# dojo-sim/Dojo.jl

Hardware: NVIDIA H100
Metric: env-steps/sec (forward step!) (higher is better)
Workload: dtype f64

## Files before the change

dojo.jl_b200/csrc/dojo_b200.cu:

```cuda
#include <cuda_runtime.h>

#include <algorithm>
#include <climits>
#include <cstdio>
#include <cstdlib>
#include <cstring>
#include <string>
#include <vector>

#include "../../include/dojo_b200.h"
#include "dojo_step_kernel.cuh"
#include "dojo_kin.cuh"
#include "dojo_kinjac.cuh"
#include "dojo_envs.cuh"
#include "dojo_storage.cuh"

using namespace dj;

extern "C" __attribute__((visibility("hidden"))) const void* dojo_cm_step_kernel(int grad);
static const void* step_kernel_fn(bool any_contact, bool grad, bool plan_smem, bool small = false) {
  if (any_contact) return dojo_cm_step_kernel(grad ? 1 : 0);
  if (plan_smem && !getenv("DOJO_B200_GENERIC_PLAN")) {
    if (!grad && small) return (const void*)dojo_step_kernel<false, true, false, true>;
    return grad ? (const void*)dojo_step_kernel<true, true> : (const void*)dojo_step_kernel<false, true>;
// ... 447 lines not shown
            gfold.push_back(joints[j].gv_off);
          }
        const BodyDev& B = bodies[b];
        const JointDev& J = joints[pj[b]];
        {
          HStep h; std::memset(&h, 0, sizeof(h));
          ElimStep& s = h.s;
          s.d_off = B.D_off; s.n = 6; s.vec_off = B.sol_off; s.r_off = B.r_off; s.nnb = 0;
          s.fold_off = (int)ilist.size(); s.fold_cnt = (int)fold.size();
          for (int f : fold) ilist.push_back(f);
          s.gfold_off = (int)ilist.size();
          for (int f : gfold) ilist.push_back(f);
          int ij = -1, ip = -1;
          if (joint_nq(J) > 0) {
            ij = s.nnb++;
            s.nb[ij].n = joint_nq(J); s.nb[ij].vec_off = J.sol_off; s.nb[ij].r_off = J.r_off; s.nb[ij].gv_off = -1; s.nb[ij].fwd_abs = -1; s.nb[ij].L_off = J.Uc_off; s.nb[ij].U_off = J.Lc_off; s.nb[ij].U_k = 6; s.nb[ij].U_row = 0;
            s.nb[ij].ld = joint_nq(J); s.nb[ij].row0 = 0;
          }
          int r0 = 0;
          if (J.parent >= 0 && J.BBpc_off >= 0) {
            ip = s.nnb++;
            const BodyDev& Pb = bodies[J.parent];
            r0 = (J.flags & JF_FULL) ? 0 : 3;
            s.nb[ip].n = 6 - r0; s.nb[ip].vec_off = Pb.sol_off + r0; s.nb[ip].r_off = Pb.r_off + r0; s.nb[ip].gv_off = J.gv_off; s.nb[ip].fwd_abs = J.S_off + 36 + r0;
            s.nb[ip].L_off = J.BBpc_off; s.nb[ip].U_off = J.BBcp_off; s.nb[ip].U_k = 6 - r0; s.nb[ip].U_row = r0;
            s.nb[ip].ld = 6; s.nb[ip].row0 = r0;
          }
          if (ij >= 0) s.tgt[ij][ij] = J.D_off;
          if (ip >= 0) s.tgt[ip][ip] = J.S_off + 7 * r0;
          if (ij >= 0 && ip >= 0) { s.tgt[ij][ip] = J.Up_off + r0; s.tgt[ip][ij] = J.Lp_off + r0 * joint_nq(J); }
          h.height = hb; h.group = -1; h.cost = 4.0 + joint_nq(J) * 0.3;
          hs.push_back(h);
        }
        int hj = hb;
        if (joint_nq(J) > 0) {
          HStep h; std::memset(&h, 0, sizeof(h));
          ElimStep& s = h.s;
          s.d_off = J.D_off; s.n = joint_nq(J); s.vec_off = J.sol_off; s.r_off = J.r_off; s.nnb = 0;
          if (J.parent >= 0) {
            const BodyDev& Pb = bodies[J.parent];
            s.nnb = 1;
            s.nb[0].n = 6; s.nb[0].vec_off = Pb.sol_off; s.nb[0].r_off = Pb.r_off; s.nb[0].gv_off = J.gv_off; s.nb[0].fwd_abs = J.S_off + 36; s.nb[0].L_off = J.Lp_off; s.nb[0].U_off = J.Up_off; s.nb[0].U_k = joint_nq(J); s.nb[0].U_row = 0;
            s.nb[0].ld = 6; s.nb[0].row0 = 0;
            s.tgt[0][0] = J.S_off;
          }
          hj = hb + 1;
          h.height = hj; h.group = -1; h.cost = 2.0 + joint_nq(J) * 0.4;
          hs.push_back(h);
        }
        return hj;
      }
    } rec{joints, bodies, contacts, parent_joint, done, hs, ilist, Ne, Ni};
    for (int j = 0; j < Ne; ++j) if (joints[j].parent < 0 && !done[joints[j].child]) rec.visit(joints[j].child);
    for (int b = 0; b < Nb; ++b) if (!done[b]) { delete h; return fail("mechanism is not a tree rooted at the origin"); }
  }
  int nphase = 0;
  for (auto& x : hs) nphase = std::max(nphase, x.height + 1);
  std::vector<ElimStep> steps;
  std::vector<int> sched((size_t)nphase * nw * 2, 0);
  for (int ph = 0; ph < nphase; ++ph) {
    std::vector<std::vector<int>> per_warp(nw);
    std::vector<double> load(nw, 0.0);
    std::vector<int> group_warp(Nb, -1);
    for (int i = 0; i < (int)hs.size(); ++i) {
      if (hs[i].height != ph) continue;
      int w;
      if (hs[i].group >= 0 && group_warp[hs[i].group] >= 0) w = group_warp[hs[i].group];
      else {
        w = 0;
        for (int k = 1; k < nw; ++k) if (load[k] < load[w]) w = k;
        if (hs[i].group >= 0) group_warp[hs[i].group] = w;
      }
      per_warp[w].push_back(i);
      load[w] += hs[i].cost;
    }
    for (int w = 0; w < nw; ++w) {
      sched[2 * (ph * nw + w)] = (int)steps.size();
      sched[2 * (ph * nw + w) + 1] = (int)per_warp[w].size();
      for (int i : per_warp[w]) steps.push_back(hs[i].s);
    }
  }
  P.nphase = nphase;
  h->nsteps = (int)steps.size();

  cudaDeviceProp prop;
  if (cudaGetDeviceProperties(&prop, device) != cudaSuccess) { delete h; g_create_error = "cudaGetDeviceProperties failed"; return DOJO_ECUDA; }
  h->sm_count = prop.multiProcessorCount;
  if (h->arena_bytes > (size_t)prop.sharedMemPerBlockOptin) {
    delete h;
    g_create_error = "dojo_create: mechanism does not fit the per-environment shared-memory arena";
    return DOJO_ENOMEM;
  }
  auto upload = [&](const void* src, size_t bytes, void** dst) -> bool {
    if (bytes == 0) { *dst = nullptr; return true; }
    if (cudaMalloc(dst, bytes) != cudaSuccess) return false;
    return cudaMemcpy(*dst, src, bytes, cudaMemcpyHostToDevice) == cudaSuccess;
  };
  std::vector<char> blob;
  {
    const void* src[8] = {bodies.data(), joints.data(), contacts.data(), steps.data(), sched.data(), ilist.data(), roles.data(), ucol.data()};
    const size_t len[8] = {sizeof(BodyDev) * Nb, sizeof(JointDev) * Ne, sizeof(ContactDev) * Ni, sizeof(ElimStep) * steps.size(), sizeof(int) * sched.size(),
                           sizeof(int) * ilist.size(), sizeof(WarpRole) * roles.size(), sizeof(int) * ucol.size()};
    const int order[8] = {3, 4, 5, 6, 7, 0, 2, 1};
    for (int q = 0; q < 8; ++q) {
      const int k = order[q];
      h->blob_off[k] = (int)blob.size();
      blob.insert(blob.end(), (const char*)src[k], (const char*)src[k] + len[k]);
      blob.resize((blob.size() + 15) & ~size_t(15), 0);
      h->blob_end[k] = (int)blob.size();
    }
    h->blob_bytes = (int)blob.size();
  }
  bool ok = upload(blob.data(), blob.size(), (void**)&h->d_blob);
  {
    std::vector<int> order;
    std::vector<char> placed(Nb, 0), used(Ne, 0);
    for (bool progress = true; progress && (int)order.size() < Ne;) {
      progress = false;
      for (int j = 0; j < Ne; ++j)
        if (!used[j] && (joints[j].parent < 0 || placed[joints[j].parent])) { order.push_back(j); used[j] = 1; placed[joints[j].child] = 1; progress = true; }
    }
    ok = ok && (int)order.size() == Ne && upload(order.data(), sizeof(int) * Ne, (void**)&h->d_kin_order);
  }
  ok = ok && cudaMalloc((void**)&h->d_counter, sizeof(int)) == cudaSuccess;
  ok = ok && cudaMalloc((void**)&h->d_order, sizeof(int) * max_batch) == cudaSuccess && cudaMalloc((void**)&h->d_prev_iters, sizeof(int32_t) * max_batch) == cudaSuccess &&
       cudaMemset(h->d_prev_iters, 0, sizeof(int32_t) * max_batch) == cudaSuccess;
  if (const char* e = getenv("DOJO_B200_LPT")) { h->lpt = atoi(e) != 0; h->lpt_mode = atoi(e); }
  ok = ok && cudaMalloc((void**)&h->d_key, sizeof(int32_t) * max_batch) == cudaSuccess;
  ok = ok && cudaMalloc((void**)&h->d_prof, (32 + 2 * (size_t)max_batch) * sizeof(unsigned long long)) == cudaSuccess && cudaMemset(h->d_prof, 0, 32 * sizeof(unsigned long long)) == cudaSuccess &&
       cudaMemset(h->d_prof + 31, 0xff, sizeof(unsigned long long)) == cudaSuccess;
  ok = ok && cudaStreamCreateWithFlags(&h->stream, cudaStreamNonBlocking) == cudaSuccess;
  ok = ok && cudaEventCreateWithFlags(&h->ev_last, cudaEventDisableTiming) == cudaSuccess;
  auto pick_slots = [&](size_t bytes) {
    int g = (int)std::min<size_t>((size_t)prop.sharedMemPerBlockOptin / bytes, (size_t)(256 / (32 * nw)));
    g = std::max(1, std::min(g, 8));
    if (const char* e = getenv("DOJO_B200_SLOTS")) { int v = atoi(e); if (v >= 1 && v <= g) g = v; }
    return g;
  };
  h->slots = pick_slots(h->arena_bytes);
  const bool smem_plan = !getenv("DOJO_B200_GLOBAL_PLAN");
  auto plan_prefix = [&](int n, size_t bytes, int* off, int* pbytes, int* mask) {
    *off = -1; *pbytes = 0; *mask = 0;
    if (!smem_plan) return;
    const size_t room = (size_t)prop.sharedMemPerBlockOptin - 1024 - n * bytes;
    for (int k = 0; k < 8; ++k)
      if ((size_t)h->blob_end[k] <= room) { *mask |= 1 << k; *pbytes = std::max(*pbytes, h->blob_end[k]); }
    for (int k = 0; k < 8; ++k)
      if (((*mask >> k) & 1) && h->blob_end[k] > *pbytes) *mask &= ~(1 << k);
    if (*mask) *off = (int)(n * bytes / sizeof(double));
  };
  plan_prefix(h->slots, h->arena_bytes, &h->plan_smem_off, &h->plan_smem_bytes, &h->plan_smem_mask);
  h->smem_fwd = h->slots * h->arena_bytes + h->plan_smem_bytes;
  h->small_step = small_step_ok(h, h->plan_smem_mask);
  h->k_fwd = step_kernel_fn(h->any_contact, false, h->plan_smem_mask == 0xff, h->small_step);
  h->k_grad = step_kernel_fn(h->any_contact, true, false);
  ok = ok && max_shared_memory(h->k_fwd, device) == cudaSuccess;
  const bool grad_fits = h->grad_bytes <= (size_t)prop.sharedMemPerBlockOptin;
  if (grad_fits) {
    h->slots_grad = pick_slots(h->grad_bytes);
    plan_prefix(h->slots_grad, h->grad_bytes, &h->plan_smem_off_grad, &h->plan_smem_bytes_grad, &h->plan_smem_mask_grad);
    h->smem_grad = h->slots_grad * h->grad_bytes + h->plan_smem_bytes_grad;
    h->k_grad = step_kernel_fn(h->any_contact, true, h->plan_smem_mask_grad == 0xff);
    ok = ok && max_shared_memory(h->k_grad, device) == cudaSuccess;
  } else h->grad_bytes = 0;
  if (!ok) { g_create_error = std::string("dojo_create: device allocation failed: ") + cudaGetErrorString(cudaGetLastError()); dojo_destroy(h); return DOJO_ECUDA; }
  P.bodies = (const BodyDev*)(h->d_blob + h->blob_off[0]); P.joints = (const JointDev*)(h->d_blob + h->blob_off[1]);
  P.contacts = (const ContactDev*)(h->d_blob + h->blob_off[2]); P.steps = (const ElimStep*)(h->d_blob + h->blob_off[3]);
  P.sched = (const int*)(h->d_blob + h->blob_off[4]); P.ilist = (const int*)(h->d_blob + h->blob_off[5]);
  P.roles = (const WarpRole*)(h->d_blob + h->blob_off[6]); P.ucol = (const int*)(h->d_blob + h->blob_off[7]);
  int occ = 1;
  cudaOccupancyMaxActiveBlocksPerMultiprocessor(&occ, h->k_fwd, 32 * h->nw * h->slots, h->smem_fwd);
  h->envs_per_sm = std::max(1, occ);
  if (h->grad_bytes) { occ = 1; cudaOccupancyMaxActiveBlocksPerMultiprocessor(&occ, h->k_grad, 32 * h->nw * h->slots_grad, h->smem_grad); h->envs_per_sm_grad = std::max(1, occ); }
  *out = h;
  return DOJO_OK;
}

extern "C" int dojo_destroy(DojoHandle* h) {
  if (!h) return DOJO_OK;
  cudaSetDevice(h->device);
  cudaFree(h->d_key); cudaFree(h->d_order); cudaFree(h->d_prev_iters); cudaFree(h->d_prof); cudaFree(h->d_blob); cudaFree(h->d_counter); cudaFree(h->d_kin_order); cudaFree(h->d_kjws); cudaFree(h->d_kjout); cudaFree(h->d_recZ[0]); cudaFree(h->d_recZ[1]); cudaFree(h->d_recS); cudaFree(h->d_recD); cudaFree(h->d_recAny); cudaFree(h->d_envTheta); cudaFree(h->d_envNorm); cudaFree(h->d_envS); cudaFree(h->d_envSn); cudaFree(h->d_envA); cudaFree(h->d_envR); cudaFree(h->d_envS0); cudaFree(h->d_envDone); cudaFree(h->d_X); cudaFree(h->d_Xn); cudaFree(h->d_gsol); cudaFree(h->d_gstatus); cudaFree(h->d_done); cudaFree(h->d_trace);
  for (int k = 0; k < 2; ++k) { cudaFree(h->d_Fz[k]); cudaFree(h->d_Fu[k]); if (h->ev_kernel[k]) cudaEventDestroy(h->ev_kernel[k]); if (h->ev_copy[k]) cudaEventDestroy(h->ev_copy[k]); }
  if (h->copy_stream) cudaStreamDestroy(h->copy_stream);
  cudaFree(h->d_Z); cudaFree(h->d_U); cudaFree(h->d_F); cudaFree(h->d_Zn); cudaFree(h->d_sol); cudaFree(h->d_status); cudaFree(h->d_iters);
  if (h->p_in) cudaFreeHost(h->p_in);
  if (h->p_out) cudaFreeHost(h->p_out);
// ... 1245 lines not shown
```

dojo.jl_b200/csrc/dojo_kernels.cuh:

```cuda
#pragma once
#include "dojo_linalg.cuh"
#include "dojo_plan.h"

namespace dj {

#ifdef DJ_ANY_CONTACT
#define DJ_SLOT_OFF(raw) ((raw) & 0x3fffffff)
#define DJ_SLOT_FULL(raw) (((raw) >> 30) & 1)
#else
#define DJ_SLOT_OFF(raw) (raw)
#endif
#ifdef DJ_ANY_CONTACT
DJ_DEV int contact_type(const ContactDev& cd) { return cd.tn & 0xff; }
DJ_DEV int contact_nh(const ContactDev& cd) { return cd.tn >> 8; }
#endif

DJ_DEV V3 ld3(const double* p) { return V3{p[0], p[1], p[2]}; }
DJ_DEV void st3(double* p, V3 v) { p[0] = v.x; p[1] = v.y; p[2] = v.z; }
DJ_DEV void add3(double* p, V3 v) { p[0] += v.x; p[1] += v.y; p[2] += v.z; }
DJ_DEV M33 ldm33(const double* p) {
  M33 r;
#pragma unroll
  for (int i = 0; i < 3; ++i)
#pragma unroll
    for (int j = 0; j < 3; ++j) r.m[i][j] = p[3 * i + j];
  return r;
}
DJ_DEV void stm33(double* p, const M33& a) {
#pragma unroll
  for (int i = 0; i < 3; ++i)
#pragma unroll
    for (int j = 0; j < 3; ++j) p[3 * i + j] = a.m[i][j];
}
DJ_DEV Quat ldq(const double* p) { return Quat{p[0], p[1], p[2], p[3]}; }

struct Ctx {
  double* A;
  const Plan* P;
  const BodyDev* bodies;
  const JointDev* joints;
  const ContactDev* contacts;
  const ElimStep* steps;
  const int* sched;
  const int* ilist;
  const WarpRole* roles;
  const int* ucol;
  int tid, nthreads, warp, lane;
  int sd;
  int bar;
  double mu;
  int slot, nslots, slot_stride;
  double* arena0;
  int* s_int;
  double* s_dbl;
  int apar, assist;
#ifdef DJ_PROFILE
  long long t_eval_jac, t_eval_ls, t_fact, t_solve, t_misc, t_align, t_cone, t_center, t_rolewait, t_last;
  long long f_fold, f_inv, f_rm, f_schur, f_bar, f_last;
#endif
};
#ifdef DJ_PROFILE
#define DJ_TICK(c, field) { long long _t = clock64(); (c).field += _t - (c).t_last; (c).t_last = _t; }
#define DJ_FTICK(c, field) { long long _t = clock64(); (c).field += _t - (c).f_last; (c).f_last = _t; }
#else
#define DJ_TICK(c, field) {}
#define DJ_FTICK(c, field) {}
#endif

#ifdef DJ_HOSTEMU
DJ_DEV void slot_sync(const Ctx& c) { hostemu_bar_sync(c.bar, c.nthreads); }
#else
DJ_DEV void slot_sync(const Ctx& c) { asm volatile("bar.sync %0, %1;" ::"r"(c.bar), "r"(c.nthreads) : "memory"); }
#endif

constexpr int kMaxAssistTrials = 16;
struct AlignInfo { int n_live, owner; };
#ifdef DJ_HOSTEMU
DJ_DEV void cta_barrier() { __syncthreads(); }
#else
__device__ __noinline__ void cta_barrier() { __syncthreads(); }
#endif
DJ_DEV AlignInfo cta_align(Ctx& c, bool live) {
  int* fl = c.s_int + 8 + 8 * c.apar;
  c.apar ^= 1;
  if (c.tid == 0) fl[c.slot] = live ? 1 : 0;
  cta_barrier();
  AlignInfo r;
  r.n_live = 0; r.owner = -1;
  for (int q = 0; q < c.nslots; ++q)
    if (fl[q]) { r.n_live++; r.owner = q; }
  return r;
}
DJ_DEV void assist_release(Ctx& c) {
  if (!c.assist) return;
  if (c.tid == 0) c.s_int[24] = 0;
  cta_barrier();
  c.assist = 0;
}

template <bool SMALL>
DJ_DEV int slot_warps(const Ctx& c) { return SMALL ? 2 : c.P->nw; }

template <bool SMALL = false>
DJ_DEV void block_nanmax2(const Ctx& c, double& a, double& b) {
  double* red = c.A + c.P->red_off;
  a = warp_nanmax(a);
  b = warp_nanmax(b);
  if (slot_warps<SMALL>(c) == 1) return;
  if (c.lane == 0) { red[2 * c.warp] = a; red[2 * c.warp + 1] = b; }
  slot_sync(c);
  a = red[0]; b = red[1];
  for (int w = 1; w < slot_warps<SMALL>(c); ++w) { a = nanmax(a, red[2 * w]); b = nanmax(b, red[2 * w + 1]); }
  slot_sync(c);
}
template <bool SMALL = false>
DJ_DEV double block_min(const Ctx& c, double a) {
  double* red = c.A + c.P->red_off;
  a = warp_min(a);
  if (slot_warps<SMALL>(c) == 1) return a;
  if (c.lane == 0) red[c.warp] = a;
  slot_sync(c);
  a = red[0];
  for (int w = 1; w < slot_warps<SMALL>(c); ++w) a = fmin(a, red[w]);
  slot_sync(c);
  return a;
}
template <bool SMALL = false>
DJ_DEV void block_sum3(const Ctx& c, double& a, double& b, double& d) {
  double* red = c.A + c.P->red_off;
  a = warp_sum(a); b = warp_sum(b); d = warp_sum(d);
  if (slot_warps<SMALL>(c) == 1) return;
  if (c.lane == 0) { red[3 * c.warp] = a; red[3 * c.warp + 1] = b; red[3 * c.warp + 2] = d; }
  slot_sync(c);
  a = red[0]; b = red[1]; d = red[2];
  for (int w = 1; w < slot_warps<SMALL>(c); ++w) { a += red[3 * w]; b += red[3 * w + 1]; d += red[3 * w + 2]; }
  slot_sync(c);
}

DJ_DEV int role_item(const WarpRole& r, int p, int lane) { return lane < r.count[p] ? r.first[p] + lane : -1; }

struct Kin {
// ... 941 lines not shown
      const double* s = A + DJ_SLOT_OFF(c.ilist[bd.g_off + g]);
      add3(rb, ld3(s));
      add3(rb + 3, ld3(s + 3));
      if (JAC) {
#ifdef DJ_ANY_CONTACT
        if (g < bd.g_ncontact || DJ_SLOT_FULL(c.ilist[bd.g_off + g])) {
#else
        if (g < bd.g_ncontact) {
#endif
#pragma unroll
          for (int i = 0; i < 36; ++i) D[i] -= s[6 + i];
        } else {
#pragma unroll
          for (int i = 0; i < 3; ++i)
#pragma unroll
            for (int j = 0; j < 3; ++j) D[(3 + i) * 6 + 3 + j] -= s[6 + 3 * i + j];
        }
      }
    }
#pragma unroll
    for (int i = 0; i < 6; ++i) rv = nanmax(rv, fabs(rb[i]));
  }
  block_nanmax2<SMALL>(c, rv, bv);
  rvio = rv;
  bvio = bv;
  slot_sync(c);
}

template <bool SMALL = false>
DJ_DEV void evaluate_ls(Ctx& c, double* W, double fk, bool pair, double& rvA, double& bvA, double& rvB, double& bvB) {
  const Plan& P = *c.P;
  double* A = c.A;
  const WarpRole& role = c.roles[c.warp];
  const bool pl = SMALL || P.ls_pair != 0;
  const int half = pl ? (c.lane >> 4) : 0;
  const int ln = pl ? (c.lane & 15) : c.lane;
  const bool on = (half == 0) || pair;
  const double f = half ? 0.5 * fk : fk;
  double* res = W + (half ? P.ls_res2_off : P.sav_off);
  c.sd = (int)(W - A) + (half ? P.ls_slot_delta : 0);
  double rv = 0.0, bv = 0.0;
  for (int p = 0; p < role.npass; ++p) {
    const int idx = on ? role_item(role, p, ln) : -1;
    if (idx < 0) continue;
    if (role.type[p] == ROLE_BODY) eval_body<false>(c, idx, f, res);
    else if (role.type[p] == ROLE_CONTACT) eval_contact<false>(c, idx, f, res, rv, bv);
    else eval_joint<false>(c, idx, f, res, rv, bv);
  }
  slot_sync(c);
  for (int p = 0; p < role.npass; ++p) {
    const int idx = on ? role_item(role, p, ln) : -1;
    if (idx < 0 || role.type[p] != ROLE_BODY) continue;
    const BodyDev& bd = c.bodies[idx];
    double* rb = res + bd.sol_off;
    for (int g = 0; g < bd.g_cnt; ++g) {
      const double* s = A + DJ_SLOT_OFF(c.ilist[bd.g_off + g]) + c.sd;
      add3(rb, ld3(s));
      add3(rb + 3, ld3(s + 3));
    }
#pragma unroll
    for (int i = 0; i < 6; ++i) rv = nanmax(rv, fabs(rb[i]));
  }
  c.sd = 0;
#pragma unroll
  for (int o = 8; o > 0; o >>= 1) {
    rv = nanmax(rv, __shfl_xor_sync(0xffffffffu, rv, o));
    bv = nanmax(bv, __shfl_xor_sync(0xffffffffu, bv, o));
  }
  if (!pl) {
    rv = nanmax(rv, __shfl_xor_sync(0xffffffffu, rv, 16));
    bv = nanmax(bv, __shfl_xor_sync(0xffffffffu, bv, 16));
  }
  double* red = W + P.red_off;
  if ((c.lane & 15) == 0) { red[4 * c.warp + 2 * (c.lane >> 4)] = rv; red[4 * c.warp + 2 * (c.lane >> 4) + 1] = bv; }
  slot_sync(c);
  rvA = red[0]; bvA = red[1]; rvB = red[2]; bvB = red[3];
  for (int w = 1; w < slot_warps<SMALL>(c); ++w) {
    rvA = nanmax(rvA, red[4 * w]); bvA = nanmax(bvA, red[4 * w + 1]);
    rvB = nanmax(rvB, red[4 * w + 2]); bvB = nanmax(bvB, red[4 * w + 3]);
  }
  slot_sync(c);
}

template <bool SMALL = false>
DJ_DEV bool factorize(Ctx& c) {
  const Plan& P = *c.P;
  double* A = c.A;
  bool ok = true;
  const int half = c.lane >> 4, l = c.lane & 15;
  const unsigned mask = 0xffffu << (16 * half);
#ifdef DJ_PROFILE
  c.f_last = clock64();
#endif
  for (int ph = 0; ph < P.nphase; ++ph) {
    const int s0 = c.sched[2 * (ph * slot_warps<SMALL>(c) + c.warp)], sn = c.sched[2 * (ph * slot_warps<SMALL>(c) + c.warp) + 1];
    for (int s = s0 + half; s < s0 + sn; s += 2) {
      const ElimStep& st = c.steps[s];
      double* Dc = A + st.d_off;
      if (st.fold_cnt > 0) {
        for (int t = l; t < st.n * st.n; t += 16) {
          double acc = Dc[t];
          for (int k = 0; k < st.fold_cnt; ++k) acc += A[c.ilist[st.fold_off + k] + t];
          Dc[t] = acc;
        }
        __syncwarp(mask);
      }
      DJ_FTICK(c, f_fold)
      ok = block_inverse(Dc, st.n, st.n, l, mask) && ok;
      DJ_FTICK(c, f_inv)
      for (int i = 0; i < st.nnb; ++i) right_multiply_inplace(A + st.nb[i].L_off, Dc, st.nb[i].n, st.n, l, mask);
      DJ_FTICK(c, f_rm)
      for (int i = 0; i < st.nnb; ++i)
        for (int j = 0; j < st.nnb; ++j)
          schur_update(A + st.tgt[i][j], st.nb[j].ld, A + st.nb[i].L_off + st.nb[j].U_row, st.n, A + st.nb[j].U_off, st.nb[i].n, st.nb[j].U_k,
                       st.nb[j].n, l, mask);
      DJ_FTICK(c, f_schur)
    }
    slot_sync(c);
    DJ_FTICK(c, f_bar)
  }
  int* flag = (int*)(A + P.red_off);
  const bool wok = __all_sync(0xffffffffu, ok);
  if (c.lane == 0) flag[c.warp] = wok ? 1 : 0;
  slot_sync(c);
  bool all = true;
  for (int w = 0; w < slot_warps<SMALL>(c); ++w) all = all && (flag[w] != 0);
  slot_sync(c);
  return all;
}

DJ_DEV double dot6(const double* a, const double* b, int n) {
  double e = 0.0, o = 0.0;
#pragma unroll
  for (int k = 0; k < 6; k += 2) {
    if (k < n) e = fma(a[k], b[k], e);
    if (k + 1 < n) o = fma(a[k + 1], b[k + 1], o);
  }
  return e + o;
}

template <bool SMALL = false>
DJ_DEV void solve(Ctx& c, int vec_off) {
  const Plan& P = *c.P;
  double* A = c.A;
  double* x = A + vec_off;
  const int lane = c.lane;
  const int half = lane >> 4, l = lane & 15;
  const int sub = l >> 3, li = l & 7;
  const WarpRole& role = c.roles[c.warp];
  for (int p = 0; p < role.npass; ++p) {
    const int idx = role_item(role, p, lane);
    if (idx < 0) continue;
    if (role.type[p] == ROLE_CONTACT) condense_contact(c, idx, x);
    else if (role.type[p] == ROLE_JOINT) condense_joint(c, idx, x);
  }
  slot_sync(c);
  for (int p = 0; p < role.npass; ++p) {
    const int idx = role_item(role, p, lane);
    if (idx < 0 || role.type[p] != ROLE_BODY) continue;
    const BodyDev& bd = c.bodies[idx];
    double* xb = x + bd.sol_off;
    for (int g = 0; g < bd.g_cnt; ++g) {
      const double* s = A + DJ_SLOT_OFF(c.ilist[bd.g_off + g]);
      add3(xb, ld3(s));
      add3(xb + 3, ld3(s + 3));
    }
  }
  slot_sync(c);
  for (int ph = 0; ph < P.nphase; ++ph) {
    const int s0 = c.sched[2 * (ph * slot_warps<SMALL>(c) + c.warp)], sn = c.sched[2 * (ph * slot_warps<SMALL>(c) + c.warp) + 1];
    for (int it = 0; 2 * it < sn; ++it) {
      const bool act = 2 * it + half < sn;
      const ElimStep& st = c.steps[s0 + 2 * it + (act ? half : 0)];
      double* xc = x + st.vec_off;
      if (act && st.fold_cnt > 0 && l < st.n) {
        double acc = xc[l];
        for (int k = 0; k < st.fold_cnt; ++k) {
          double* v = A + c.ilist[st.fold_off + k] + 36;
          acc += v[l];
          v[l] = 0.0;
        }
        xc[l] = acc;
      }
      __syncwarp();
      if (act && sub < st.nnb && li < st.nb[sub].n) {
        const ElimNb& nb = st.nb[sub];
        const double* L = A + nb.L_off + li * st.n;
        const double acc = dot6(L, xc, st.n);
        double* tgt = nb.fwd_abs >= 0 ? A + nb.fwd_abs : x + nb.vec_off;
        tgt[li] -= acc;
      }
      __syncwarp();
    }
    slot_sync(c);
  }
  for (int ph = P.nphase - 1; ph >= 0; --ph) {
    const int s0 = c.sched[2 * (ph * slot_warps<SMALL>(c) + c.warp)], sn = c.sched[2 * (ph * slot_warps<SMALL>(c) + c.warp) + 1];
    for (int it = (sn + 1) / 2 - 1; it >= 0; --it) {
      const bool act = 2 * it + half < sn;
      const ElimStep& st = c.steps[s0 + 2 * it + (act ? half : 0)];
      const double* Dc = A + st.d_off;
      double* xc = x + st.vec_off;
      if (act && st.nnb > 0 && l < st.n) {
        double acc = 0.0;
        for (int j = 0; j < st.nnb; ++j) {
          const ElimNb& nb = st.nb[j];
          int r = l - nb.U_row;
          if (r >= 0 && r < nb.U_k) {
            acc += dot6(A + nb.U_off + r * nb.n, x + nb.vec_off, nb.n);
          }
        }
        xc[l] -= acc;
      }
      __syncwarp();
      double acc = 0.0;
      if (act && l < st.n) acc = dot6(Dc + l * st.n, xc, st.n);
      __syncwarp();
      if (act && l < st.n) xc[l] = acc;
      __syncwarp();
    }
    slot_sync(c);
  }
  for (int p = 0; p < role.npass; ++p) {
    const int idx = role_item(role, p, lane);
    if (idx < 0) continue;
    if (role.type[p] == ROLE_CONTACT) recover_contact(c, idx, x);
    else if (role.type[p] == ROLE_JOINT) recover_joint(c, idx, x);
  }
  slot_sync(c);
}

DJ_DEV double ort_step(double lam, double dl, double tau) { return dl < 0.0 ? fmin(1.0, -tau * lam / dl) : 1.0; }
DJ_DEV double soc_step(double l0, double l1, double l2, double d0, double d1, double d2, double tau) {
  const double eps = 1e-14;
  double ll = fmax(l0 * l0 - (l1 * l1 + l2 * l2), 1e-25) + eps;
  double ld = l0 * d0 - (l1 * d1 + l2 * d2) + eps;
  double rs = ld / ll;
  double sq = sqrt(ll);
  double fct = (ld / sq + d0) / (l0 / sq + 1.0);
  double r1 = d1 / sq - fct * l1 / ll;
  double r2 = d2 / sq - fct * l2 / ll;
  double nr = sqrt(r1 * r1 + r2 * r2);
  return (nr - rs > 0.0) ? fmin(1.0, tau / (nr - rs)) : 1.0;
}
template <bool SMALL = false>
DJ_DEV double cone_line_search(Ctx& c, double tau_ort, double tau_soc) {
  const Plan& P = *c.P;
  const double* sol = c.A + P.sol_off;
  const double* dl = c.A + P.rhs_off;
  const WarpRole& role = c.roles[c.warp];
  double a = 1.0;
  for (int p = 0; p < role.npass; ++p) {
#ifndef DJ_ANY_CONTACT
    if (role.type[p] == ROLE_CONTACT && role.count[p] <= 16) {
      const int ci = c.lane >> 1;
      if (ci < role.count[p]) {
        const ContactDev& cd = c.contacts[role.first[p] + ci];
        const int o = cd.sol_off + 4 * (c.lane & 1);
        const double* v = sol + o;
        const double* dv = dl + o;
        a = fmin(a, ort_step(v[0], dv[0], tau_ort));
        a = fmin(a, soc_step(v[1], v[2], v[3], dv[1], dv[2], dv[3], tau_soc));
      }
      continue;
    }
#endif
    const int idx = role_item(role, p, c.lane);
    if (idx < 0) continue;
    if (role.type[p] == ROLE_CONTACT) {
      const ContactDev& cd = c.contacts[idx];
      const double* s = sol + cd.sol_off;
#ifdef DJ_ANY_CONTACT
      if (contact_type(cd) != 2) {
        const int n2 = 2 * contact_nh(cd);
        for (int i = 0; i < n2; ++i) a = fmin(a, ort_step(s[i], dl[cd.sol_off + i], tau_ort));
        continue;
      }
#endif
      const double* g = s + 4;
      const double* ds = dl + cd.sol_off;
      const double* dg = ds + 4;
      a = fmin(a, ort_step(s[0], ds[0], tau_ort));
      a = fmin(a, ort_step(g[0], dg[0], tau_ort));
      a = fmin(a, soc_step(s[1], s[2], s[3], ds[1], ds[2], ds[3], tau_soc));
      a = fmin(a, soc_step(g[1], g[2], g[3], dg[1], dg[2], dg[3], tau_soc));
    } else if (role.type[p] == ROLE_JOINT) {
      const JointDev& jd = c.joints[idx];
      for (int i = 0; i < 2 * jd.nb_r; ++i) a = fmin(a, ort_step(sol[jd.sol_off + jd.ne + i], dl[jd.sol_off + jd.ne + i], tau_ort));
    }
  }
  return block_min<SMALL>(c, a);
}

template <bool SMALL = false>
DJ_DEV void centering(Ctx& c, double aaff, double& nu, double& nuaff) {
  const Plan& P = *c.P;
  const double* sol = c.A + P.sol_off;
  const double* dl = c.A + P.rhs_off;
  const WarpRole& role = c.roles[c.warp];
  double sn = 0.0, sa = 0.0, cnt = 0.0;
  for (int p = 0; p < role.npass; ++p) {
    const int idx = role_item(role, p, c.lane);
    if (idx < 0) continue;
    if (role.type[p] == ROLE_CONTACT) {
      const ContactDev& cd = c.contacts[idx];
#ifdef DJ_ANY_CONTACT
      if (contact_type(cd) != 2) {
        const int nh = contact_nh(cd);
        for (int i = 0; i < nh; ++i) {
          double s = sol[cd.sol_off + i], g = sol[cd.sol_off + nh + i];
          sn += s * g;
          sa += (s + aaff * dl[cd.sol_off + i]) * (g + aaff * dl[cd.sol_off + nh + i]);
// ... 230 lines not shown
```

dojo.jl_b200/csrc/dojo_plan.h:

```cpp
#pragma once
#include <stdint.h>

namespace dj {

constexpr double kReg = 1.0e-10;
constexpr int kSlot = 15;
constexpr int kSlotC = 42;
constexpr int kScratch = 42;
constexpr int kLim = 12;

enum RoleType { ROLE_BODY = 0, ROLE_CONTACT = 1, ROLE_JOINT = 2 };

struct BodyDev {
  double mass;
  double J[9];
  int sol_off;
  int st_off;
  int cst_off;
  int D_off;
  int g_off, g_cnt, g_ncontact;
  int pjoint;
  int cj_off, cj_cnt;
  int ct_off, ct_cnt;
  int r_off;
  int gb_off;
};

struct JointDev {
  int parent, child;
  int n, sol_off;
  int ne;
  int nl_t, nl_r, nb2_r, nb_r;
  int lim_off;
  int nfree_t, nfree_r, u_off;
  int flags;
  double pa[3], pb[3], qoff[4];
  double Ct[9], At[9], Cr[9], Ar[9];
  double spring_r, damper_r, spring_off_r[3], lo[3], hi[3];
  int D_off;
  int Uc_off, Lc_off;
  int Up_off, Lp_off, Gp_off;
  int BBpc_off, BBcp_off;
  int slot_c, slot_p;
  int S_off;
  int r_off;
  int gj_off;
  int gv_off;
};

enum JointFlags {
  JF_TRA_SPRING = 1,
  JF_TRA_DAMPER = 2,
  JF_LIM_TRA = 4,
  JF_FULL = 8
};
static_assert(sizeof(JointDev) == 568, "JointDev layout is part of the kernels' addressing");
#if defined(__CUDACC__) || defined(DJ_HOSTEMU)
#define DJ_PLAN_FN __host__ __device__ inline
#else
#define DJ_PLAN_FN inline
#endif
DJ_PLAN_FN int joint_nq(const JointDev& j) { return j.ne + j.nb2_r; }
DJ_PLAN_FN const double* joint_tra_params(const JointDev& j) { return j.Ct + 3 * j.nl_t; }
DJ_PLAN_FN double* joint_tra_params(JointDev& j) { return j.Ct + 3 * j.nl_t; }

struct ContactDev {
  int body, sol_off;
  double mu, radius;
  double n[3], t[6], o[3], off[3];
  int J_off, G_off, rec_off;
  int slot;
  int gc_off;
  int tn;
};
static_assert(sizeof(ContactDev) == 168, "ContactDev layout is part of the kernels' addressing");

struct ElimNb {
  int n, vec_off;
  int r_off;
  int gv_off;
  int fwd_abs;
  int L_off;
  int U_off, U_k;
  int U_row;
  int ld;
  int row0;
};
struct ElimStep {
  int d_off, n, vec_off;
  int r_off;
  int gfold_off;
  int nnb;
  ElimNb nb[2];
  int tgt[2][2];
  int fold_off, fold_cnt;
};

struct WarpRole {
  int npass;
  int type[3], first[3], count[3];
};

struct Plan {
  int Nb, Ne, Ni, nres, nu, nz;
  int nw;
  int nphase;
  int ls_pair, ls_slot_delta, ls_res2_off;
  int ls_assist;
  int jpair;
  double h, input_scaling, g[3];
  int sol_off, rhs_off, sav_off, red_off, mat_off, mat_len, arena_len;
  const BodyDev* bodies;
  const JointDev* joints;
  const ContactDev* contacts;
  const ElimStep* steps;
  const int* sched;
  const int* ilist;
  const WarpRole* roles;
  int n_red;
  int ncol;
  int ch;
  int gvec_off;
  int grad_len;
  const int* ucol;
};

struct Options {
  double rtol, btol, undercut, no_progress_undercut;
  int max_iter, max_ls, no_progress_max;
};

}
```

dojo.jl_b200/csrc/dojo_step_kernel.cuh:

```cuda
#pragma once
#include "../../include/dojo_b200.h"
#include "dojo_grad.cuh"

namespace dj {

struct StepArgs {
  Plan plan;
  Options opts;
  int B;
  const double* Z;
  const double* U;
  const double* Fext;
  double* Zn;
  double* sol;
  int32_t* status;
  int32_t* iters;
  int* done_count;
  int* done_list;
  double* sol_raw;
  double* Fz;
  double* Fu;
  double* Fc;
  uint32_t flags;
  int* counter;
// ... 27 lines not shown
#pragma unroll
    for (int i = 0; i < 13; ++i) o[i] = v[i];
    for (int r = 0; r < n_peers; ++r) {
      double* po = peer[r] + peer_off + 13 * c.tid;
#pragma unroll
      for (int i = 0; i < 13; ++i) po[i] = v[i];
    }
  }
}

#ifndef DJ_LB_THREADS
#define DJ_LB_THREADS 256
#define DJ_LB_BLOCKS 1
#endif
#ifdef DJ_PROFILE
__device__ __forceinline__ unsigned long long k_t0g(unsigned long long* prof) { return *((volatile unsigned long long*)(prof + 31)); }
#endif
template <bool GRAD, bool PLAN_SMEM = false, bool TRACE = false, bool SMALL = false, bool REC = false>
__global__ void __launch_bounds__(DJ_LB_THREADS, DJ_LB_BLOCKS) dojo_step_kernel(const StepArgs a) {
  static_assert(!SMALL || (!GRAD && PLAN_SMEM && !TRACE), "SMALL is a specialisation of the untraced forward kernel with the plan in shared memory");
  static_assert(!REC || (!GRAD && !TRACE && !SMALL), "REC is a variant of the generic untraced forward kernel");
  extern __shared__ double arena[];
  __shared__ __align__(8) int s_env[128];
  const int slot_threads = 32 * (SMALL ? 2 : a.plan.nw);
  const int slot = threadIdx.x / slot_threads;
  Ctx c;
  c.A = arena + (size_t)slot * a.slot_stride;
  c.P = &a.plan;
  c.tid = threadIdx.x - slot * slot_threads;
  c.nthreads = slot_threads;
  c.warp = c.tid >> 5;
  c.lane = c.tid & 31;
  c.bar = 1 + slot;
  c.sd = 0;
  c.mu = 0.0;
  c.slot = slot; c.nslots = blockDim.x / slot_threads; c.slot_stride = a.slot_stride; c.arena0 = arena;
  c.s_int = s_env; c.s_dbl = reinterpret_cast<double*>(s_env + 32);
  c.apar = 0; c.assist = 0;
  {
    const char* gb = a.plan_blob;
    const char* sb = nullptr;
    if (PLAN_SMEM || a.plan_smem_off >= 0) {
      int4* dst = reinterpret_cast<int4*>(arena + a.plan_smem_off);
      const int4* src = reinterpret_cast<const int4*>(a.plan_blob);
#ifndef DJ_HOSTEMU
      __shared__ __align__(8) unsigned long long s_plan_bar;
      const unsigned bar = (unsigned)__cvta_generic_to_shared(&s_plan_bar);
      if (threadIdx.x == 0) {
        asm volatile("mbarrier.init.shared::cta.b64 [%0], 1;" ::"r"(bar) : "memory");
        asm volatile("fence.proxy.async.shared::cta;" ::: "memory");
      }
      __syncthreads();
      if (threadIdx.x == 0) {
        const unsigned bytes = (unsigned)a.plan_smem_bytes;
        asm volatile("mbarrier.arrive.expect_tx.shared::cta.b64 _, [%0], %1;" ::"r"(bar), "r"(bytes) : "memory");
        asm volatile("cp.async.bulk.shared::cluster.global.mbarrier::complete_tx::bytes [%0], [%1], %2, [%3];"
                     ::"r"((unsigned)__cvta_generic_to_shared(dst)), "l"(src), "r"(bytes), "r"(bar) : "memory");
      }
      {
        unsigned done = 0;
        while (!done)
          asm volatile("{ .reg .pred p; mbarrier.try_wait.parity.shared::cta.b64 p, [%1], 0; selp.u32 %0, 1, 0, p; }" : "=r"(done) : "r"(bar) : "memory");
      }
#else
      for (int i = threadIdx.x; i < a.plan_smem_bytes / 16; i += blockDim.x) dst[i] = src[i];
      __syncthreads();
#endif
      sb = reinterpret_cast<const char*>(dst);
    }
#define DJ_TABLE(k) ((PLAN_SMEM || (sb && ((a.plan_smem_mask >> (k)) & 1))) ? sb + a.plan_off[k] : gb + a.plan_off[k])
    c.bodies = reinterpret_cast<const BodyDev*>(DJ_TABLE(0));
    c.joints = reinterpret_cast<const JointDev*>(DJ_TABLE(1));
    c.contacts = reinterpret_cast<const ContactDev*>(DJ_TABLE(2));
    c.steps = reinterpret_cast<const ElimStep*>(DJ_TABLE(3));
    c.sched = reinterpret_cast<const int*>(DJ_TABLE(4));
    c.ilist = reinterpret_cast<const int*>(DJ_TABLE(5));
    c.roles = reinterpret_cast<const WarpRole*>(DJ_TABLE(6));
    c.ucol = reinterpret_cast<const int*>(DJ_TABLE(7));
#undef DJ_TABLE
  }
#ifdef DJ_PROFILE
  c.t_eval_jac = c.t_eval_ls = c.t_fact = c.t_solve = c.t_misc = c.t_align = c.t_cone = c.t_center = c.t_rolewait = 0; c.t_last = clock64();
  c.f_fold = c.f_inv = c.f_rm = c.f_schur = c.f_bar = 0;
  long long k_c0 = clock64(); unsigned long long k_t0; asm volatile("mov.u64 %0, %%globaltimer;" : "=l"(k_t0));
  int k_envs = 0;
  if (c.tid == 0 && a.prof) atomicMin(a.prof + 31, k_t0);
#endif
  if (!GRAD) asm volatile("griddepcontrol.launch_dependents;" ::: "memory");
  const Plan& P = a.plan;
  for (;;) {
    if (c.tid == 0) {
      int q = atomicAdd(a.counter, 1);
      int env = (q < a.B && a.order) ? a.order[q] : q;
      if (GRAD && a.done_list && q < a.B) {
        while ((env = ((volatile int*)a.done_list)[q]) < 0) __nanosleep(256);
        __threadfence();
      }
      s_env[slot] = env;
    }
    slot_sync(c);
    const int e = s_env[slot];
    slot_sync(c);
    if (e >= a.B) break;
    DJ_TICK(c, t_misc)
#ifdef DJ_PROFILE
    k_envs++;
    unsigned long long e_t0; asm volatile("mov.u64 %0, %%globaltimer;" : "=l"(e_t0));
#endif
    const double* z = a.Z + (size_t)e * P.nz;
    int worst = 0, iters = 0, status = 0;
    if (!GRAD) {
      for (int t = 0; t < a.T; ++t) {
        const double* u = a.U ? a.U + ((size_t)t * a.B + e) * P.nu : nullptr;
        const double* fx = a.Fext ? a.Fext + (size_t)e * 6 * P.Nb : nullptr;
        prologue(c, z, u, fx, false);
        status = mehrotra<TRACE, SMALL>(c, a.opts, &iters, TRACE ? a.trace + (size_t)e * max(a.opts.max_iter, 0) * 5 : nullptr);
        worst = max(worst, status);
        double* zo = (a.traj ? a.traj + ((size_t)t * a.B + e) * P.nz : a.Zn + (size_t)e * P.nz);
        epilogue(c, zo, (a.flags & DOJO_FLAG_Q1_LITERAL_RETURN) != 0, (t + 1 == a.T) ? a.n_peers : 0, a.peer_buf, a.gather_off + (long long)e * P.nz);
        if (REC) {
          const size_t p = (size_t)t * a.B + e;
          for (int k = c.tid; k < P.nres; k += c.nthreads) a.sol_raw[p * P.nres + k] = c.A[P.sol_off + k];
          if (c.tid == 0) {
            a.status[p] = status;
            if (a.iters) a.iters[p] = iters;
          }
          if (a.done_list) {
            __threadfence();
            slot_sync(c);
            if (c.tid == 0) {
              const int pos = atomicAdd(a.done_count, 1);
              __threadfence();
              ((volatile int*)a.done_list)[pos] = (int)p;
            }
          }
        }
        if (t + 1 < a.T) { __threadfence_block(); slot_sync(c); z = zo; }
      }
      if (a.traj && !REC) {
        slot_sync(c);
        for (int k = c.tid; k < P.nz; k += c.nthreads) a.Zn[(size_t)e * P.nz + k] = a.traj[((size_t)(a.T - 1) * a.B + e) * P.nz + k];
      }
      status = worst;
      if (a.sol_raw && !REC)
        for (int t = c.tid; t < P.nres; t += c.nthreads) a.sol_raw[(size_t)e * P.nres + t] = c.A[P.sol_off + t];
    } else {
      const double* u = a.U ? a.U + (size_t)e * P.nu : nullptr;
      const double* fx = a.Fext ? a.Fext + (size_t)e * 6 * P.Nb : nullptr;
      prologue(c, z, u, fx, true);
      for (int t = c.tid; t < P.nres; t += c.nthreads) c.A[P.sol_off + t] = a.sol_raw[(size_t)e * P.nres + t];
      slot_sync(c);
      double rv, bv;
      c.mu = 0.0;
      evaluate<true>(c, 0.0, P.rhs_off, rv, bv);
      if (a.flags & DOJO_FLAG_Q2_LITERAL_GRADIENTS) {
        if (c.tid < P.Nb) {
          const BodyDev& bd = c.bodies[c.tid];
          Kin k = body_kin(c, c.tid, 0.0);
          double* stp = c.A + bd.st_off;
          st3(stp, k.x3);
          stp[3] = k.q3.s; stp[4] = k.q3.x; stp[5] = k.q3.y; stp[6] = k.q3.z;
          st3(c.A + bd.gb_off + 27, k.w);
        }
        slot_sync(c);
      }
      status = a.status ? a.status[e] : 0;
      const size_t ng = 12 * (size_t)P.Nb;
      if (!gradients(c, a.Fz + (size_t)e * ng * ng, a.Fu + (size_t)e * ng * P.nu, a.Fc ? a.Fc + (size_t)e * ng * 5 * P.Ni : nullptr) && status == 0) status = 3;
    }
    if (a.sol) {
      double* so = a.sol + (size_t)e * P.nres;
      const int first_body = c.bodies[0].sol_off;
      for (int t = c.tid; t < P.nres; t += c.nthreads)
        if (t >= first_body) so[t] = c.A[P.sol_off + t];
      if (c.tid < P.Ne) {
        const JointDev& jd = c.joints[c.tid];
        const double* src = c.A + P.sol_off + jd.sol_off;
        double* dst = so + jd.sol_off;
#ifdef DJ_ANY_CONTACT
        if (jd.flags & JF_LIM_TRA) {
          for (int i = 0; i < 2 * jd.nb_r; ++i) dst[i] = src[jd.ne + i];
          for (int i = 0; i < jd.ne; ++i) dst[2 * jd.nb_r + i] = src[i];
        } else
#endif
        {
        for (int i = 0; i < jd.nl_t; ++i) dst[i] = src[i];
        for (int i = 0; i < 2 * jd.nb_r; ++i) dst[jd.nl_t + i] = src[jd.ne + i];
        for (int i = 0; i < jd.nl_r; ++i) dst[jd.nl_t + 2 * jd.nb_r + i] = src[jd.nl_t + i];
        }
      }
    }
    if (c.tid == 0) {
      if (a.status && !REC) a.status[e] = status;
      if (!GRAD && !REC) {
        if (a.iters) a.iters[e] = iters;
        if (a.prev_iters) a.prev_iters[e] = iters;
      }
#ifdef DJ_PROFILE
      if (a.prof) { unsigned long long e_t1; asm volatile("mov.u64 %0, %%globaltimer;" : "=l"(e_t1)); a.prof[32 + 2 * e] = e_t0 - k_t0g(a.prof); a.prof[33 + 2 * e] = e_t1 - e_t0; }
#endif
    }
    if (!GRAD && !REC && a.done_list) {
      __threadfence();
      slot_sync(c);
      if (c.tid == 0) {
        const int pos = atomicAdd(a.done_count, 1);
        __threadfence();
        ((volatile int*)a.done_list)[pos] = e;
      }
    }
    slot_sync(c);
  }
  for (;;) {
    const AlignInfo ai = cta_align(c, false);
    if (ai.n_live == 0) break;
    if (!GRAD && P.ls_assist && ai.n_live == 1 && a.opts.max_ls <= kMaxAssistTrials) ls_assist_loop<SMALL>(c, a.opts, ai.owner, slot < ai.owner ? slot + 1 : slot);
  }
  if (!GRAD && a.n_peers > 0) {
    if (threadIdx.x == 0) {
      __threadfence_system();
      for (int r = 0; r < a.n_peers; ++r) atomicAdd_system(a.peer_flag[r], 1ull);
    }
  }
  if (GRAD) asm volatile("griddepcontrol.wait;" ::: "memory");
#ifdef DJ_PROFILE
  DJ_TICK(c, t_misc)
  if (c.lane == 0 && a.prof) atomicAdd(a.prof + 17 + c.warp, (unsigned long long)c.t_rolewait);
  if (c.tid == 0 && a.prof) {
    atomicAdd(a.prof + 0, (unsigned long long)c.t_eval_jac); atomicAdd(a.prof + 1, (unsigned long long)c.t_eval_ls);
    atomicAdd(a.prof + 2, (unsigned long long)c.t_fact); atomicAdd(a.prof + 3, (unsigned long long)c.t_solve); atomicAdd(a.prof + 4, (unsigned long long)c.t_misc);
    atomicAdd(a.prof + 5, (unsigned long long)c.f_fold); atomicAdd(a.prof + 6, (unsigned long long)c.f_inv); atomicAdd(a.prof + 7, (unsigned long long)c.f_rm);
    atomicAdd(a.prof + 8, (unsigned long long)c.f_schur); atomicAdd(a.prof + 9, (unsigned long long)c.f_bar);
    unsigned long long k_t1; asm volatile("mov.u64 %0, %%globaltimer;" : "=l"(k_t1));
    atomicMax(a.prof + 10, (unsigned long long)(clock64() - k_c0)); atomicMax(a.prof + 11, k_t1 - k_t0);
    atomicMax(a.prof + 12, (unsigned long long)k_envs); atomicAdd(a.prof + 13, (unsigned long long)(clock64() - k_c0));
    atomicAdd(a.prof + 14, (unsigned long long)c.t_align); atomicAdd(a.prof + 15, (unsigned long long)c.t_cone); atomicAdd(a.prof + 16, (unsigned long long)c.t_center);
  }
#endif
}


}
```

Baseline: 461,900.

## Encode block LDU elimination steps as compact packed per-warp op program

Host setup now compiles each warp's elimination steps into 48-byte packed records with 16-bit offsets, inline fold sources, and per-warp contiguous ordering. This program is appended to the sched table and placed first in the plan blob. Factorize and the forward/backward solves read these records as int4 loads instead of walking larger ElimStep structs and indirect sched/ilist lookups. The aim is to cut plan-table memory traffic and shared-memory footprint in the inner solver. The trade-offs are extra bit unpacking and a create-time failure when offsets exceed 16 bits. Profiling counters for the solve phases are also added.

```diff
diff --git a/dojo.jl_b200/csrc/dojo_b200.cu b/dojo.jl_b200/csrc/dojo_b200.cu
--- a/dojo.jl_b200/csrc/dojo_b200.cu
+++ b/dojo.jl_b200/csrc/dojo_b200.cu
@@ -553,6 +553,48 @@
   }
   P.nphase = nphase;
   h->nsteps = (int)steps.size();
+  {
+    std::vector<int> cnt((size_t)nphase * nw), wfirst(nw);
+    std::vector<LduOp> ops;
+    bool fits = true;
+    auto u16 = [&](int v) { fits = fits && v >= 0 && v < kLduNone; return v & 0xffff; };
+    auto u8 = [&](int v) { fits = fits && v >= 0 && v < 256; return v & 0xff; };
+    for (int w = 0; w < nw; ++w) {
+      wfirst[w] = (int)ops.size();
+      for (int ph = 0; ph < nphase; ++ph) {
+        const int s0 = sched[2 * (ph * nw + w)], sn = sched[2 * (ph * nw + w) + 1];
+        cnt[ph * nw + w] = sn;
+        for (int s = s0; s < s0 + sn; ++s) {
+          const ElimStep& st = steps[s];
+          int f[kLduFold] = {0, 0, 0};
+          for (int k = 0; k < std::min(st.fold_cnt, kLduFold); ++k) f[k] = ilist[st.fold_off + k];
+          LduOp op;
+          std::memset(&op, 0, sizeof(op));
+          op.w[0] = u16(st.d_off) | u16(st.vec_off) << 16;
+          op.w[1] = u8(st.n) | u8(st.nnb) << 8 | u16(st.fold_cnt) << 16;
+          op.w[2] = u16(st.fold_off) | u16(f[0]) << 16;
+          op.w[3] = u16(f[1]) | u16(f[2]) << 16;
+          for (int i = 0; i < st.nnb; ++i) {
+            const ElimNb& nb = st.nb[i];
+            int* q = op.w + 4 * (1 + i);
+            q[0] = u16(nb.L_off) | (nb.fwd_abs >= 0 ? u16(nb.fwd_abs) : kLduNone) << 16;
+            q[1] = u16(nb.vec_off) | u16(nb.U_off) << 16;
+            q[2] = u8(nb.n) | u8(nb.U_row) << 8 | u8(nb.U_k) << 16 | u8(nb.ld) << 24;
+            q[3] = u16(st.tgt[i][0]) | (st.nnb > 1 ? u16(st.tgt[i][1]) : 0) << 16;
+          }
+          ops.push_back(op);
+        }
+      }
+    }
+    if (!fits) { delete h; return fail("the block LDU program does not fit its 16-bit offsets"); }
+    P.prog_cnt = (int)sched.size();
+    sched.insert(sched.end(), cnt.begin(), cnt.end());
+    sched.insert(sched.end(), wfirst.begin(), wfirst.end());
+    sched.resize((sched.size() + 3) & ~size_t(3), 0);
+    P.prog_ops = (int)sched.size();
+    const int* words = reinterpret_cast<const int*>(ops.data());
+    sched.insert(sched.end(), words, words + ops.size() * (sizeof(LduOp) / sizeof(int)));
+  }
 
   cudaDeviceProp prop;
   if (cudaGetDeviceProperties(&prop, device) != cudaSuccess) { delete h; g_create_error = "cudaGetDeviceProperties failed"; return DOJO_ECUDA; }
@@ -572,7 +614,7 @@
     const void* src[8] = {bodies.data(), joints.data(), contacts.data(), steps.data(), sched.data(), ilist.data(), roles.data(), ucol.data()};
     const size_t len[8] = {sizeof(BodyDev) * Nb, sizeof(JointDev) * Ne, sizeof(ContactDev) * Ni, sizeof(ElimStep) * steps.size(), sizeof(int) * sched.size(),
                            sizeof(int) * ilist.size(), sizeof(WarpRole) * roles.size(), sizeof(int) * ucol.size()};
-    const int order[8] = {3, 4, 5, 6, 7, 0, 2, 1};
+    const int order[8] = {4, 3, 5, 6, 7, 0, 2, 1};
     for (int q = 0; q < 8; ++q) {
       const int k = order[q];
       h->blob_off[k] = (int)blob.size();
diff --git a/dojo.jl_b200/csrc/dojo_kernels.cuh b/dojo.jl_b200/csrc/dojo_kernels.cuh
--- a/dojo.jl_b200/csrc/dojo_kernels.cuh
+++ b/dojo.jl_b200/csrc/dojo_kernels.cuh
@@ -57,6 +57,7 @@
 #ifdef DJ_PROFILE
   long long t_eval_jac, t_eval_ls, t_fact, t_solve, t_misc, t_align, t_cone, t_center, t_rolewait, t_last;
   long long f_fold, f_inv, f_rm, f_schur, f_bar, f_last;
+  long long s_cond, s_fwd, s_bwd, s_rec, s_bar;
 #endif
 };
 #ifdef DJ_PROFILE
@@ -1164,6 +1165,13 @@
   slot_sync(c);
 }
 
+DJ_DEV const int* ldu_cnt(const Ctx& c) { return c.sched + c.P->prog_cnt; }
+DJ_DEV const int4* ldu_op(const Ctx& c, int k) { return reinterpret_cast<const int4*>(c.sched + c.P->prog_ops) + 3 * k; }
+DJ_DEV int ldu_fold(const Ctx& c, int4 h, int j) {
+  return j == 0 ? hi16(h.z) : j == 1 ? lo16(h.w) : j == 2 ? hi16(h.w) : c.ilist[lo16(h.z) + j];
+}
+static_assert(kLduFold == 3, "ldu_fold names three inline fold sources");
+
 template <bool SMALL = false>
 DJ_DEV bool factorize(Ctx& c) {
   const Plan& P = *c.P;
@@ -1171,33 +1179,44 @@
   bool ok = true;
   const int half = c.lane >> 4, l = c.lane & 15;
   const unsigned mask = 0xffffu << (16 * half);
+  const int nw = slot_warps<SMALL>(c);
+  const int* cnt = ldu_cnt(c);
+  int k = cnt[P.nphase * nw + c.warp];
 #ifdef DJ_PROFILE
   c.f_last = clock64();
 #endif
   for (int ph = 0; ph < P.nphase; ++ph) {
-    const int s0 = c.sched[2 * (ph * slot_warps<SMALL>(c) + c.warp)], sn = c.sched[2 * (ph * slot_warps<SMALL>(c) + c.warp) + 1];
-    for (int s = s0 + half; s < s0 + sn; s += 2) {
-      const ElimStep& st = c.steps[s];
-      double* Dc = A + st.d_off;
-      if (st.fold_cnt > 0) {
-        for (int t = l; t < st.n * st.n; t += 16) {
+    const int sn = cnt[ph * nw + c.warp];
+    for (int s = half; s < sn; s += 2) {
+      const int4* q = ldu_op(c, k + s);
+      const int4 h = q[0];
+      const int n = byte_of(h.y, 0), nnb = byte_of(h.y, 1), fold_cnt = hi16(h.y);
+      double* Dc = A + lo16(h.x);
+      if (fold_cnt > 0) {
+        for (int t = l; t < n * n; t += 16) {
           double acc = Dc[t];
-          for (int k = 0; k < st.fold_cnt; ++k) acc += A[c.ilist[st.fold_off + k] + t];
+          for (int j = 0; j < fold_cnt; ++j) acc += A[ldu_fold(c, h, j) + t];
           Dc[t] = acc;
         }
         __syncwarp(mask);
       }
       DJ_FTICK(c, f_fold)
-      ok = block_inverse(Dc, st.n, st.n, l, mask) && ok;
+      ok = block_inverse(Dc, n, n, l, mask) && ok;
       DJ_FTICK(c, f_inv)
-      for (int i = 0; i < st.nnb; ++i) right_multiply_inplace(A + st.nb[i].L_off, Dc, st.nb[i].n, st.n, l, mask);
+      for (int i = 0; i < nnb; ++i) {
+        const int4 a = q[1 + i];
+        right_multiply_inplace(A + lo16(a.x), Dc, byte_of(a.z, 0), n, l, mask);
+      }
       DJ_FTICK(c, f_rm)
-      for (int i = 0; i < st.nnb; ++i)
-        for (int j = 0; j < st.nnb; ++j)
-          schur_update(A + st.tgt[i][j], st.nb[j].ld, A + st.nb[i].L_off + st.nb[j].U_row, st.n, A + st.nb[j].U_off, st.nb[i].n, st.nb[j].U_k,
-                       st.nb[j].n, l, mask);
+      for (int i = 0; i < nnb; ++i)
+        for (int j = 0; j < nnb; ++j) {
+          const int4 ai = q[1 + i], aj = q[1 + j];
+          schur_update(A + (j ? hi16(ai.w) : lo16(ai.w)), byte_of(aj.z, 3), A + lo16(ai.x) + byte_of(aj.z, 1), n, A + hi16(aj.y), byte_of(ai.z, 0),
+                       byte_of(aj.z, 2), byte_of(aj.z, 0), l, mask);
+        }
       DJ_FTICK(c, f_schur)
     }
+    k += sn;
     slot_sync(c);
     DJ_FTICK(c, f_bar)
   }
@@ -1230,13 +1249,18 @@
   const int half = lane >> 4, l = lane & 15;
   const int sub = l >> 3, li = l & 7;
   const WarpRole& role = c.roles[c.warp];
+#ifdef DJ_PROFILE
+  c.f_last = clock64();
+#endif
   for (int p = 0; p < role.npass; ++p) {
     const int idx = role_item(role, p, lane);
     if (idx < 0) continue;
     if (role.type[p] == ROLE_CONTACT) condense_contact(c, idx, x);
     else if (role.type[p] == ROLE_JOINT) condense_joint(c, idx, x);
   }
-  slot_sync(c);
+  DJ_FTICK(c, s_cond)
+  slot_sync(c);
+  DJ_FTICK(c, s_bar)
   for (int p = 0; p < role.npass; ++p) {
     const int idx = role_item(role, p, lane);
     if (idx < 0 || role.type[p] != ROLE_BODY) continue;
@@ -1248,60 +1272,77 @@
       add3(xb + 3, ld3(s + 3));
     }
   }
-  slot_sync(c);
+  DJ_FTICK(c, s_cond)
+  slot_sync(c);
+  DJ_FTICK(c, s_bar)
+  const int nw = slot_warps<SMALL>(c);
+  const int* cnt = ldu_cnt(c);
+  int k = cnt[P.nphase * nw + c.warp];
   for (int ph = 0; ph < P.nphase; ++ph) {
-    const int s0 = c.sched[2 * (ph * slot_warps<SMALL>(c) + c.warp)], sn = c.sched[2 * (ph * slot_warps<SMALL>(c) + c.warp) + 1];
+    const int sn = cnt[ph * nw + c.warp];
     for (int it = 0; 2 * it < sn; ++it) {
       const bool act = 2 * it + half < sn;
-      const ElimStep& st = c.steps[s0 + 2 * it + (act ? half : 0)];
-      double* xc = x + st.vec_off;
-      if (act && st.fold_cnt > 0 && l < st.n) {
+      const int4* q = ldu_op(c, k + 2 * it + (act ? half : 0));
+      const int4 h = q[0];
+      const int n = byte_of(h.y, 0), fold_cnt = hi16(h.y);
+      double* xc = x + hi16(h.x);
+      if (act && fold_cnt > 0 && l < n) {
         double acc = xc[l];
-        for (int k = 0; k < st.fold_cnt; ++k) {
-          double* v = A + c.ilist[st.fold_off + k] + 36;
+        for (int j = 0; j < fold_cnt; ++j) {
+          double* v = A + ldu_fold(c, h, j) + 36;
           acc += v[l];
           v[l] = 0.0;
         }
         xc[l] = acc;
       }
       __syncwarp();
-      if (act && sub < st.nnb && li < st.nb[sub].n) {
-        const ElimNb& nb = st.nb[sub];
-        const double* L = A + nb.L_off + li * st.n;
-        const double acc = dot6(L, xc, st.n);
-        double* tgt = nb.fwd_abs >= 0 ? A + nb.fwd_abs : x + nb.vec_off;
-        tgt[li] -= acc;
+      if (act && sub < byte_of(h.y, 1)) {
+        const int4 a = q[1 + sub];
+        if (li < byte_of(a.z, 0)) {
+          const double* L = A + lo16(a.x) + li * n;
+          const double acc = dot6(L, xc, n);
+          double* tgt = hi16(a.x) != kLduNone ? A + hi16(a.x) : x + lo16(a.y);
+          tgt[li] -= acc;
+        }
       }
       __syncwarp();
     }
+    k += sn;
+    DJ_FTICK(c, s_fwd)
     slot_sync(c);
+    DJ_FTICK(c, s_bar)
   }
   for (int ph = P.nphase - 1; ph >= 0; --ph) {
-    const int s0 = c.sched[2 * (ph * slot_warps<SMALL>(c) + c.warp)], sn = c.sched[2 * (ph * slot_warps<SMALL>(c) + c.warp) + 1];
+    const int sn = cnt[ph * nw + c.warp];
+    k -= sn;
     for (int it = (sn + 1) / 2 - 1; it >= 0; --it) {
       const bool act = 2 * it + half < sn;
-      const ElimStep& st = c.steps[s0 + 2 * it + (act ? half : 0)];
-      const double* Dc = A + st.d_off;
-      double* xc = x + st.vec_off;
-      if (act && st.nnb > 0 && l < st.n) {
+      const int4* q = ldu_op(c, k + 2 * it + (act ? half : 0));
+      const int4 h = q[0];
+      const int n = byte_of(h.y, 0), nnb = byte_of(h.y, 1);
+      const double* Dc = A + lo16(h.x);
+      double* xc = x + hi16(h.x);
+      if (act && nnb > 0 && l < n) {
         double acc = 0.0;
-        for (int j = 0; j < st.nnb; ++j) {
-          const ElimNb& nb = st.nb[j];
-          int r = l - nb.U_row;
-          if (r >= 0 && r < nb.U_k) {
-            acc += dot6(A + nb.U_off + r * nb.n, x + nb.vec_off, nb.n);
+        for (int j = 0; j < nnb; ++j) {
+          const int4 a = q[1 + j];
+          const int nn = byte_of(a.z, 0), r = l - byte_of(a.z, 1);
+          if (r >= 0 && r < byte_of(a.z, 2)) {
+            acc += dot6(A + hi16(a.y) + r * nn, x + lo16(a.y), nn);
           }
         }
         xc[l] -= acc;
       }
       __syncwarp();
       double acc = 0.0;
-      if (act && l < st.n) acc = dot6(Dc + l * st.n, xc, st.n);
+      if (act && l < n) acc = dot6(Dc + l * n, xc, n);
       __syncwarp();
-      if (act && l < st.n) xc[l] = acc;
+      if (act && l < n) xc[l] = acc;
       __syncwarp();
     }
+    DJ_FTICK(c, s_bwd)
     slot_sync(c);
+    DJ_FTICK(c, s_bar)
   }
   for (int p = 0; p < role.npass; ++p) {
     const int idx = role_item(role, p, lane);
@@ -1309,7 +1350,9 @@
     if (role.type[p] == ROLE_CONTACT) recover_contact(c, idx, x);
     else if (role.type[p] == ROLE_JOINT) recover_joint(c, idx, x);
   }
-  slot_sync(c);
+  DJ_FTICK(c, s_rec)
+  slot_sync(c);
+  DJ_FTICK(c, s_bar)
 }
 
 DJ_DEV double ort_step(double lam, double dl, double tau) { return dl < 0.0 ? fmin(1.0, -tau * lam / dl) : 1.0; }
diff --git a/dojo.jl_b200/csrc/dojo_plan.h b/dojo.jl_b200/csrc/dojo_plan.h
--- a/dojo.jl_b200/csrc/dojo_plan.h
+++ b/dojo.jl_b200/csrc/dojo_plan.h
@@ -96,6 +96,16 @@
   int fold_off, fold_cnt;
 };
 
+constexpr int kLduFold = 3;
+constexpr int kLduNone = 0xffff;
+struct alignas(16) LduOp {
+  int w[12];
+};
+static_assert(sizeof(LduOp) == 48, "LduOp is read as three 16-byte words");
+DJ_PLAN_FN int lo16(int v) { return v & 0xffff; }
+DJ_PLAN_FN int hi16(int v) { return (int)((unsigned)v >> 16); }
+DJ_PLAN_FN int byte_of(int v, int k) { return (v >> (8 * k)) & 0xff; }
+
 struct WarpRole {
   int npass;
   int type[3], first[3], count[3];
@@ -115,6 +125,7 @@
   const ContactDev* contacts;
   const ElimStep* steps;
   const int* sched;
+  int prog_cnt, prog_ops;
   const int* ilist;
   const WarpRole* roles;
   int n_red;
diff --git a/dojo.jl_b200/csrc/dojo_step_kernel.cuh b/dojo.jl_b200/csrc/dojo_step_kernel.cuh
--- a/dojo.jl_b200/csrc/dojo_step_kernel.cuh
+++ b/dojo.jl_b200/csrc/dojo_step_kernel.cuh
@@ -133,6 +133,7 @@
 #ifdef DJ_PROFILE
   c.t_eval_jac = c.t_eval_ls = c.t_fact = c.t_solve = c.t_misc = c.t_align = c.t_cone = c.t_center = c.t_rolewait = 0; c.t_last = clock64();
   c.f_fold = c.f_inv = c.f_rm = c.f_schur = c.f_bar = 0;
+  c.s_cond = c.s_fwd = c.s_bwd = c.s_rec = c.s_bar = 0;
   long long k_c0 = clock64(); unsigned long long k_t0; asm volatile("mov.u64 %0, %%globaltimer;" : "=l"(k_t0));
   int k_envs = 0;
   if (c.tid == 0 && a.prof) atomicMin(a.prof + 31, k_t0);
@@ -282,6 +283,8 @@
     atomicAdd(a.prof + 2, (unsigned long long)c.t_fact); atomicAdd(a.prof + 3, (unsigned long long)c.t_solve); atomicAdd(a.prof + 4, (unsigned long long)c.t_misc);
     atomicAdd(a.prof + 5, (unsigned long long)c.f_fold); atomicAdd(a.prof + 6, (unsigned long long)c.f_inv); atomicAdd(a.prof + 7, (unsigned long long)c.f_rm);
     atomicAdd(a.prof + 8, (unsigned long long)c.f_schur); atomicAdd(a.prof + 9, (unsigned long long)c.f_bar);
+    atomicAdd(a.prof + 25, (unsigned long long)c.s_cond); atomicAdd(a.prof + 26, (unsigned long long)c.s_fwd); atomicAdd(a.prof + 27, (unsigned long long)c.s_bwd);
+    atomicAdd(a.prof + 28, (unsigned long long)c.s_rec); atomicAdd(a.prof + 29, (unsigned long long)c.s_bar);
     unsigned long long k_t1; asm volatile("mov.u64 %0, %%globaltimer;" : "=l"(k_t1));
     atomicMax(a.prof + 10, (unsigned long long)(clock64() - k_c0)); atomicMax(a.prof + 11, k_t1 - k_t0);
     atomicMax(a.prof + 12, (unsigned long long)k_envs); atomicAdd(a.prof + 13, (unsigned long long)(clock64() - k_c0));
```

Result: faster. 482,500, median of 6 (+4.4%).
